# shanguanma/speaker_diarization

Hardware: AMD Instinct MI355X
Metric: diarized frames/sec (10 ms hop) (higher is better)
Workload: dtype bf16; 1 GPU; C2: AliMeeting-shaped 4-spk meeting, TS-VAD CAM++_ots_vad + 6-layer Conformer + BiLSTM (ots_vad_style v1), rs_len 6 s, shift 1 s; windows=600, global_batch=64, device_batch=640, parallelism=1 GPU

## Files before the change

### speaker_diarization_amd/csrc/mha_block.hip

```cpp
#include "common.h"
#include "kernels.h"
#include "launch.h"
#include "prof.h"

namespace sd {
namespace {

constexpr int kD = 384, kHD = 48, kNH = 8;
constexpr int kKT32 = kD / 32;
constexpr int kKC = kD / 64;
constexpr int kTP = 160;
constexpr int kTilesPerSeq = kTP / 16;
constexpr int kPR = 16;
constexpr int kSlot = kKC * kPR * 64;
constexpr int kDmaPerPiece = kKC * (kPR / 8);
constexpr int kVS = 48;
constexpr int kPieces = kNH * 3 * (kHD / kPR);
typedef __attribute__((address_space(3))) void* lds_ptr_t;

template <int SEQ, int W, int NSLOT, int QS>
struct MhaL {
  static constexpr int kTiles = SEQ * kTilesPerSeq;
  static constexpr int kMaxTiles = (kTiles + W - 1) / W;
  static constexpr int kThreads = W * 64;
  static constexpr int kSeqLds = 2 * kTP * QS + kTP * kVS;
  static constexpr size_t kSmem = sizeof(uint16_t) * ((size_t)NSLOT * kSlot + (size_t)SEQ * kSeqLds) +
                                  sizeof(float) * 3 * kD;
  static_assert(kMaxTiles == 2 || kMaxTiles == 3, "2 or 3 row tiles per wave (af registers)");
};

template <int N>
__device__ __forceinline__ void wait_vm() {
  asm volatile("s_waitcnt vmcnt(%0)" ::"n"(N) : "memory");
}

template <int SEQ, int W, int NSLOT, int QS, int PROBE = 0>
__global__ __launch_bounds__(W * 64) void mha_block_kernel(MhaBlockArgs a) {
  using L = MhaL<SEQ, W, NSLOT, QS>;
  constexpr int kTiles = L::kTiles, kMaxTiles = L::kMaxTiles, kThreads = L::kThreads, kSeqLds = L::kSeqLds;
  extern __shared__ __attribute__((aligned(1024))) uint16_t sm[];
  uint16_t* Ws = sm;
  const int tid = threadIdx.x, lane = tid & 63;
  const int w = __builtin_amdgcn_readfirstlane(tid >> 6);
  const int l15 = lane & 15, lk = lane >> 4;
  float* s_bias = reinterpret_cast<float*>(Ws + NSLOT * kSlot + SEQ * kSeqLds);
  const int T = a.T;
  const int ntile = w < kTiles - (kMaxTiles - 1) * W ? kMaxTiles : kMaxTiles - 1;
  int sqj[kMaxTiles], rowj[kMaxTiles];
#pragma unroll
  for (int j = 0; j < kMaxTiles; ++j) {
    const int t = w + W * j;
    sqj[j] = min(t, kTiles - 1) / kTilesPerSeq;
    rowj[j] = (min(t, kTiles - 1) % kTilesPerSeq) * 16 + l15;
  }
  auto qimg = [&](int sq) { return Ws + NSLOT * kSlot + sq * kSeqLds; };

  const int lrow = lane >> 3, lch = lane & 7;
  auto issue_piece = [&](int i) {
    const int h = i / 9, c = (i / 3) % 3, ft = i % 3;
    uint16_t* slot = Ws + (i % NSLOT) * kSlot;
    for (int j = w; j < kDmaPerPiece; j += W) {
      const int kc = j >> 1, rg = j & 1;
      const int r = rg * 8 + lrow;
      const uint32_t off =
          (uint32_t)((((int64_t)(c * kD + h * kHD + ft * kPR + r)) * kD + kc * 64 + ((lch ^ (r & 7)) * 8)) * 2);
      dma_lds16(reinterpret_cast<const char*>(a.W) + off, (lds_ptr_t)(slot + ((size_t)kc * kPR + rg * 8) * 64));
    }
  };
  const int my_dma = (kDmaPerPiece - w + W - 1) / W;
#pragma unroll
  for (int i = 0; i < NSLOT - 1; ++i) issue_piece(i);
  for (int i = tid; i < 3 * kD; i += kThreads) s_bias[i] = a.bias[i];
  if constexpr (QS > kHD) {
    for (int i = tid; i < SEQ * kTP * 2; i += kThreads) {
      const int q = i / (kTP * 2), r = (i >> 1) % kTP, c = kHD + (i & 1) * 8;
      uint16_t* qs = Ws + NSLOT * kSlot + q * kSeqLds;
      *reinterpret_cast<uint4*>(qs + r * QS + c) = make_uint4(0u, 0u, 0u, 0u);
      *reinterpret_cast<uint4*>(qs + kTP * QS + r * QS + c) = make_uint4(0u, 0u, 0u, 0u);
    }
  }

  bf16x8 af[kMaxTiles][kKT32];
#pragma unroll
  for (int rt = 0; rt < kMaxTiles; ++rt) {
    const int row = rowj[rt];
    const int s = blockIdx.x * SEQ + sqj[rt];
    const bool live = rt < ntile && s < a.S && row < T;
    const int64_t r = (int64_t)s * T + row;
    const uint16_t* yr = a.y_tiled ? reinterpret_cast<const uint16_t*>(a.y) + (r >> 4) * (16 * kD) + ((r & 15) + 16 * lk) * 8
                                   : reinterpret_cast<const uint16_t*>(a.y) + r * kD + 8 * lk;
    const int ks = a.y_tiled ? 512 : 32;
#pragma unroll
    for (int kk = 0; kk < kKT32; ++kk)
      af[rt][kk] = __builtin_bit_cast(bf16x8, live ? *reinterpret_cast<const uint4*>(yr + ks * kk)
                                                   : make_uint4(0u, 0u, 0u, 0u));
  }

  int klenj[SEQ];
#pragma unroll
  for (int q = 0; q < SEQ; ++q) {
    const int s = blockIdx.x * SEQ + q;
    klenj[q] = s < a.S ? (a.key_len ? min(a.key_len[s], T) : T) : 0;
  }
  const int tr_off = ((4 * lk + (l15 >> 2)) * kVS + 4 * (l15 & 3)) * 2;
  typedef short v4s __attribute__((ext_vector_type(4)));
  typedef __attribute__((address_space(3))) v4s* lds_v4s_t;
  bool drain = true;

  for (int i = 0; i < kPieces; ++i) {
    if constexpr (NSLOT == 4) {
      if (drain || i + 1 >= kPieces) wait_vm<0>();
      else if (i + 2 >= kPieces) {
        if (my_dma == 3) wait_vm<3>(); else if (my_dma == 2) wait_vm<2>(); else wait_vm<1>();
      } else {
        if (my_dma == 3) wait_vm<6>(); else if (my_dma == 2) wait_vm<4>(); else wait_vm<2>();
      }
    } else if constexpr (NSLOT == 3) {
      if (drain || i + 1 >= kPieces) wait_vm<0>();
      else if (my_dma == 3) wait_vm<3>();
      else if (my_dma == 2) wait_vm<2>();
      else wait_vm<1>();
    } else {
      static_assert(NSLOT == 2, "ring depth");
      wait_vm<0>();
    }
    drain = false;
    __syncthreads();
    if (i + NSLOT - 1 < kPieces) issue_piece(i + NSLOT - 1);
    const int h = i / 9, c = (i / 3) % 3, ft = i % 3;
    const uint16_t* slot = Ws + (i % NSLOT) * kSlot;
    floatx4 acc[kMaxTiles];
#pragma unroll
    for (int rt = 0; rt < kMaxTiles; ++rt) acc[rt] = floatx4{0.f, 0.f, 0.f, 0.f};
    auto wfrag = [&](int kk) {
      const int kc = kk >> 1, cc = (kk & 1) * 4 + lk;
      return *reinterpret_cast<const bf16x8*>(slot + (kc * kPR + l15) * 64 + ((cc ^ (l15 & 7)) * 8));
    };
    constexpr int kWPD = 3;
    bf16x8 wq[kWPD];
#pragma unroll
    for (int q = 0; q < kWPD; ++q) wq[q] = wfrag(q);
#pragma unroll
    for (int kk = 0; kk < kKT32; ++kk) {
      const bf16x8 wcur = wq[kk % kWPD];
      if (kk + kWPD < kKT32) wq[kk % kWPD] = wfrag(kk + kWPD);
      if constexpr (PROBE & 2) {
        asm volatile("" :: "v"(wcur));
        continue;
      }
      acc[0] = __builtin_amdgcn_mfma_f32_16x16x32_bf16(wcur, af[0][kk], acc[0], 0, 0, 0);
      acc[1] = __builtin_amdgcn_mfma_f32_16x16x32_bf16(wcur, af[1][kk], acc[1], 0, 0, 0);
      if constexpr (kMaxTiles > 2) {
        if (W == 4 || ntile > 2) acc[2] = __builtin_amdgcn_mfma_f32_16x16x32_bf16(wcur, af[2][kk], acc[2], 0, 0, 0);
      }
      asm volatile("" ::: "memory");
    }
    const int ld = c == 2 ? kVS : QS;
    const int coff = c * kTP * QS;
    const float scl = c == 0 ? a.scale : 1.f;
    const int n0 = ft * 16 + 4 * lk;
    const float4 bv = *reinterpret_cast<const float4*>(s_bias + c * kD + h * kHD + n0);
#pragma unroll
    for (int rt = 0; rt < kMaxTiles; ++rt)
      if (rt < ntile)
        *reinterpret_cast<uint2*>(qimg(sqj[rt]) + coff + rowj[rt] * ld + n0) =
            make_uint2(pack_bf16x2((acc[rt][0] + bv.x) * scl, (acc[rt][1] + bv.y) * scl),
                       pack_bf16x2((acc[rt][2] + bv.z) * scl, (acc[rt][3] + bv.w) * scl));
    if (c != 2 || ft != 2 || (PROBE & 1)) continue;
    __syncthreads();

#pragma unroll 1
    for (int rt = 0; rt < ntile; ++rt) {
      const int row = rowj[rt];
      const int s = blockIdx.x * SEQ + sqj[rt];
      if (s >= a.S) continue;
      const uint16_t* Qs = qimg(sqj[rt]);
      const uint16_t* Ks = Qs + kTP * QS;
      const uint16_t* Vs = Ks + kTP * QS;
      const int klen = klenj[sqj[rt]];
      bf16x8 qf[2];
#pragma unroll
      for (int kc = 0; kc < 2; ++kc) qf[kc] = *reinterpret_cast<const bf16x8*>(Qs + row * QS + kc * 32 + lk * 8);
      if constexpr (QS == kHD) {
        if (lk >= 2) qf[1] = __builtin_bit_cast(bf16x8, make_uint4(0u, 0u, 0u, 0u));
      }
      floatx4 o[3] = {{0.f, 0.f, 0.f, 0.f}, {0.f, 0.f, 0.f, 0.f}, {0.f, 0.f, 0.f, 0.f}};
      float m_run = -INFINITY, l_run = 0.f;
      for (int k0 = 0; k0 < klen; k0 += 32) {
        floatx4 sc[2];
#pragma unroll
        for (int st = 0; st < 2; ++st) {
          floatx4 sacc = {0.f, 0.f, 0.f, 0.f};
#pragma unroll
          for (int kc = 0; kc < 2; ++kc) {
            const bf16x8 kf = *reinterpret_cast<const bf16x8*>(Ks + (k0 + st * 16 + l15) * QS + kc * 32 + lk * 8);
            sacc = __builtin_amdgcn_mfma_f32_16x16x32_bf16(kf, qf[kc], sacc, 0, 0, 0);
          }
          sc[st] = sacc;
        }
        float tmax = -INFINITY;
#pragma unroll
        for (int st = 0; st < 2; ++st)
#pragma unroll
          for (int r = 0; r < 4; ++r) {
            const int key = k0 + st * 16 + lk * 4 + r;
            const float v = key < klen ? sc[st][r] : -INFINITY;
            sc[st][r] = v;
            tmax = fmaxf(tmax, v);
          }
        tmax = fmaxf(tmax, __shfl_xor(tmax, 16, 64));
        tmax = fmaxf(tmax, __shfl_xor(tmax, 32, 64));
        const float m_new = fmaxf(m_run, tmax);
        const float alpha = (m_new == -INFINITY) ? 1.f : __expf(m_run - m_new);
        float psum = 0.f;
#pragma unroll
        for (int st = 0; st < 2; ++st)
#pragma unroll
          for (int r = 0; r < 4; ++r) {
            const float pv = (m_new == -INFINITY) ? 0.f : __expf(sc[st][r] - m_new);
            sc[st][r] = pv;
            psum += pv;
          }
        psum += __shfl_xor(psum, 16, 64);
        psum += __shfl_xor(psum, 32, 64);
        l_run = l_run * alpha + psum;
        m_run = m_new;
        bf16x8 pb;
#pragma unroll
        for (int j = 0; j < 8; ++j) pb[j] = (__bf16)sc[j >> 2][j & 3];
        const uint32_t vbase = (uint32_t)reinterpret_cast<uintptr_t>((__attribute__((address_space(3))) void*)Vs) +
                               (uint32_t)(k0 * kVS * 2) + (uint32_t)tr_off;
#pragma unroll
        for (int dt = 0; dt < 3; ++dt) {
          const v4s lo = __builtin_amdgcn_ds_read_tr16_b64_v4i16((lds_v4s_t)(uintptr_t)(vbase + dt * 32));
          const v4s hi = __builtin_amdgcn_ds_read_tr16_b64_v4i16((lds_v4s_t)(uintptr_t)(vbase + 16 * kVS * 2 + dt * 32));
          const bf16x8 va = __builtin_bit_cast(bf16x8, __builtin_shufflevector(lo, hi, 0, 1, 2, 3, 4, 5, 6, 7));
#pragma unroll
          for (int r = 0; r < 4; ++r) o[dt][r] *= alpha;
          o[dt] = __builtin_amdgcn_mfma_f32_16x16x32_bf16(va, pb, o[dt], 0, 0, 0);
        }
      }
      if (row < T) {
        const float inv = l_run > 0.f ? 1.f / l_run : 0.f;
        const int64_t r = (int64_t)s * T + row;
        uint16_t* ob = reinterpret_cast<uint16_t*>(a.out);
#pragma unroll
        for (int dt = 0; dt < 3; ++dt) {
          const int f = h * kHD + dt * 16 + 4 * lk;
          const int64_t off = a.out_tiled ? (((r >> 4) * kKT32 + (f >> 5)) * 64 + (r & 15) + 16 * ((f & 31) >> 3)) * 8 + (f & 7)
                                          : r * a.ldo + f;
          *reinterpret_cast<uint2*>(ob + off) =
              make_uint2(pack_bf16x2(o[dt][0] * inv, o[dt][1] * inv), pack_bf16x2(o[dt][2] * inv, o[dt][3] * inv));
        }
        drain = true;
      }
    }
  }
}

template <int SEQ, int W, int NSLOT, int QS, int PROBE = 0>
void launch_mha(const MhaBlockArgs& a, hipStream_t st) {
  using L = MhaL<SEQ, W, NSLOT, QS>;
  allow_dynamic_lds<&mha_block_kernel<SEQ, W, NSLOT, QS, PROBE>>((int)L::kSmem);
  hipLaunchKernelGGL((mha_block_kernel<SEQ, W, NSLOT, QS, PROBE>), dim3((a.S + SEQ - 1) / SEQ), dim3(L::kThreads),
                     L::kSmem, st, a);
}

}

bool mha_block_supported(int D, int nh, int T, bool bf16) {
  static const bool off = getenv("SDIAR_NO_MHA_BLOCK") != nullptr;
  return !off && bf16 && D == kD && nh == kNH && T >= 1 && T <= kTP;
}

void mha_block(const MhaBlockArgs& a, hipStream_t st, int variant) {
  SD_CHECK(mha_block_supported(kD, a.nh, a.T, true) && a.D == kD, kErrInvalid, "mha_block: unsupported shape");
  SD_CHECK(a.ldo % 4 == 0, kErrInvalid, "mha_block: output row stride must be a multiple of 4");
  SD_CHECK(!(a.out_tiled || a.y_tiled) || ((int64_t)a.S * a.T % 16 == 0 && a.ldo == kD), kErrInvalid,
           "mha_block: the tiled layouts need S * T % 16 == 0 and ldo == D");
  if (a.S <= 0) return;
  SD_CHECK(a.y != nullptr, kErrInvalid, "mha_block: y (LayerNorm'd bf16 rows) is required");
  const double rows = (double)a.S * a.T;
  const double flops = 2.0 * rows * 3 * kD * kD + 4.0 * a.S * (double)a.T * a.T * kD;
  const double bytes = rows * kD * (2.0 + 2.0) + 2.0 * 3 * kD * kD;
  ProfScope prof("mha_block", flops, bytes, st);
  const int var = variant >= 0 ? variant : 0;
  switch (var) {
    case 1: launch_mha<2, 8, 3, 64>(a, st); break;
    case 2: launch_mha<1, 4, 2, 64>(a, st); break;
    case 3: launch_mha<1, 4, 2, 48>(a, st); break;
    case 4: launch_mha<1, 4, 3, 48>(a, st); break;
    case 5: launch_mha<1, 8, 3, 64>(a, st); break;
    case 6: launch_mha<1, 8, 2, 48>(a, st); break;
    case 7: launch_mha<2, 8, 4, 48>(a, st); break;
    case 8: launch_mha<2, 8, 3, 48, 1>(a, st); break;
    case 9: launch_mha<2, 8, 3, 48, 2>(a, st); break;
    case 10: launch_mha<2, 8, 3, 48, 3>(a, st); break;
    default: launch_mha<2, 8, 3, 48>(a, st); break;
  }
  SD_LAUNCH_CHECK();
}

}
```

Before: 2.486 million frames/s.

## Replace online softmax with two-pass exact-max attention and software-pipelined K reads

The attention inner loop now makes a first pass computing QK^T scores only to find the exact row max. A second pass then recomputes the scores, exponentiates against that fixed max and accumulates PV without any per-block rescaling of the output or running sum. K fragment loads are software-pipelined one block ahead, and sched_group_barrier hints interleave the exp VALU work with the next QK MFMAs. The row-sum reduction is deferred to the end, and output addressing is simplified to 32-bit offsets from a per-block base. In exchange the QK MFMAs are done twice.

```diff
diff --git a/speaker_diarization_amd/csrc/mha_block.hip b/speaker_diarization_amd/csrc/mha_block.hip
--- a/speaker_diarization_amd/csrc/mha_block.hip
+++ b/speaker_diarization_amd/csrc/mha_block.hip
@@ -2,6 +2,8 @@
 #include "kernels.h"
 #include "launch.h"
 #include "prof.h"
+
+#include <type_traits>
 
 namespace sd {
 namespace {
@@ -105,6 +107,9 @@
   const int tr_off = ((4 * lk + (l15 >> 2)) * kVS + 4 * (l15 & 3)) * 2;
   typedef short v4s __attribute__((ext_vector_type(4)));
   typedef __attribute__((address_space(3))) v4s* lds_v4s_t;
+  const int64_t r0 = (int64_t)blockIdx.x * SEQ * T;
+  const int r0lo = a.out_tiled ? (int)(r0 & 15) : 0;
+  uint16_t* const obase = reinterpret_cast<uint16_t*>(a.out) + (a.out_tiled ? (r0 >> 4) * (16 * kD) : r0 * a.ldo);
   bool drain = true;
 
   for (int i = 0; i < kPieces; ++i) {
@@ -185,71 +190,120 @@
         if (lk >= 2) qf[1] = __builtin_bit_cast(bf16x8, make_uint4(0u, 0u, 0u, 0u));
       }
       floatx4 o[3] = {{0.f, 0.f, 0.f, 0.f}, {0.f, 0.f, 0.f, 0.f}, {0.f, 0.f, 0.f, 0.f}};
-      float m_run = -INFINITY, l_run = 0.f;
-      for (int k0 = 0; k0 < klen; k0 += 32) {
-        floatx4 sc[2];
-#pragma unroll
-        for (int st = 0; st < 2; ++st) {
-          floatx4 sacc = {0.f, 0.f, 0.f, 0.f};
-#pragma unroll
-          for (int kc = 0; kc < 2; ++kc) {
-            const bf16x8 kf = *reinterpret_cast<const bf16x8*>(Ks + (k0 + st * 16 + l15) * QS + kc * 32 + lk * 8);
-            sacc = __builtin_amdgcn_mfma_f32_16x16x32_bf16(kf, qf[kc], sacc, 0, 0, 0);
+      const uint32_t kbase = (uint32_t)reinterpret_cast<uintptr_t>((lds_ptr_t)Ks) + (uint32_t)(l15 * QS + lk * 8) * 2;
+      const uint32_t vbase = (uint32_t)reinterpret_cast<uintptr_t>((lds_ptr_t)Vs) + (uint32_t)tr_off;
+      constexpr uint32_t kKStep = 32 * QS * 2, kVStep = 32 * kVS * 2;
+      typedef __attribute__((address_space(3))) const bf16x8* lds_bf16x8_t;
+      auto kread = [&](uint32_t ka, bf16x8 (&kf)[4]) {
+#pragma unroll
+        for (int j = 0; j < 4; ++j) kf[j] = *(lds_bf16x8_t)(uintptr_t)(ka + (uint32_t)((j >> 1) * 16 * QS + (j & 1) * 32) * 2);
+      };
+      auto smfma = [&](const bf16x8 (&kf)[4], floatx4 (&sc)[2]) {
+#pragma unroll
+        for (int st = 0; st < 2; ++st)
+          sc[st] = __builtin_amdgcn_mfma_f32_16x16x32_bf16(kf[2 * st], qf[0], floatx4{0.f, 0.f, 0.f, 0.f}, 0, 0, 0);
+#pragma unroll
+        for (int st = 0; st < 2; ++st)
+          sc[st] = __builtin_amdgcn_mfma_f32_16x16x32_bf16(kf[2 * st + 1], qf[1], sc[st], 0, 0, 0);
+      };
+      auto mask = [&](int k0, floatx4 (&sc)[2]) {
+#pragma unroll
+        for (int st = 0; st < 2; ++st)
+#pragma unroll
+          for (int r = 0; r < 4; ++r) sc[st][r] = k0 + st * 16 + lk * 4 + r < klen ? sc[st][r] : -INFINITY;
+      };
+      float l_run = 0.f;
+      if (klen > 0) {
+        float m_row = -INFINITY;
+        auto rowmax = [&](const floatx4 (&sc)[2]) {
+#pragma unroll
+          for (int st = 0; st < 2; ++st)
+#pragma unroll
+            for (int r = 0; r < 4; ++r) m_row = fmaxf(m_row, sc[st][r]);
+        };
+        bf16x8 kf[4];
+        uint32_t ka = kbase;
+        kread(ka, kf);
+        int k0 = 0;
+        for (; k0 + 32 < klen; k0 += 32) {
+          floatx4 sc[2];
+          smfma(kf, sc);
+          ka += kKStep;
+          asm volatile("" : "+v"(ka));
+          kread(ka, kf);
+          rowmax(sc);
+        }
+        {
+          floatx4 sc[2];
+          smfma(kf, sc);
+          mask(k0, sc);
+          rowmax(sc);
+        }
+        m_row = fmaxf(m_row, __shfl_xor(m_row, 16, 64));
+        m_row = fmaxf(m_row, __shfl_xor(m_row, 32, 64));
+        const bool no_max = __any(m_row == -INFINITY) != 0;
+        floatx4 scn[2];
+        ka = kbase;
+        uint32_t va = vbase;
+        kread(ka, kf);
+        smfma(kf, scn);
+        auto step = [&](int k0, auto last) {
+          constexpr bool kLast = decltype(last)::value;
+          floatx4 sc[2] = {scn[0], scn[1]};
+          if constexpr (!kLast) {
+            ka += kKStep;
+            asm volatile("" : "+v"(ka));
+            kread(ka, kf);
           }
-          sc[st] = sacc;
-        }
-        float tmax = -INFINITY;
-#pragma unroll
-        for (int st = 0; st < 2; ++st)
-#pragma unroll
-          for (int r = 0; r < 4; ++r) {
-            const int key = k0 + st * 16 + lk * 4 + r;
-            const float v = key < klen ? sc[st][r] : -INFINITY;
-            sc[st][r] = v;
-            tmax = fmaxf(tmax, v);
+          bf16x8 vf[3];
+#pragma unroll
+          for (int dt = 0; dt < 3; ++dt) {
+            const v4s lo = __builtin_amdgcn_ds_read_tr16_b64_v4i16((lds_v4s_t)(uintptr_t)(va + dt * 32));
+            const v4s hi = __builtin_amdgcn_ds_read_tr16_b64_v4i16((lds_v4s_t)(uintptr_t)(va + 16 * kVS * 2 + dt * 32));
+            vf[dt] = __builtin_bit_cast(bf16x8, __builtin_shufflevector(lo, hi, 0, 1, 2, 3, 4, 5, 6, 7));
           }
-        tmax = fmaxf(tmax, __shfl_xor(tmax, 16, 64));
-        tmax = fmaxf(tmax, __shfl_xor(tmax, 32, 64));
-        const float m_new = fmaxf(m_run, tmax);
-        const float alpha = (m_new == -INFINITY) ? 1.f : __expf(m_run - m_new);
-        float psum = 0.f;
-#pragma unroll
-        for (int st = 0; st < 2; ++st)
-#pragma unroll
-          for (int r = 0; r < 4; ++r) {
-            const float pv = (m_new == -INFINITY) ? 0.f : __expf(sc[st][r] - m_new);
-            sc[st][r] = pv;
-            psum += pv;
-          }
-        psum += __shfl_xor(psum, 16, 64);
-        psum += __shfl_xor(psum, 32, 64);
-        l_run = l_run * alpha + psum;
-        m_run = m_new;
-        bf16x8 pb;
-#pragma unroll
-        for (int j = 0; j < 8; ++j) pb[j] = (__bf16)sc[j >> 2][j & 3];
-        const uint32_t vbase = (uint32_t)reinterpret_cast<uintptr_t>((__attribute__((address_space(3))) void*)Vs) +
-                               (uint32_t)(k0 * kVS * 2) + (uint32_t)tr_off;
-#pragma unroll
-        for (int dt = 0; dt < 3; ++dt) {
-          const v4s lo = __builtin_amdgcn_ds_read_tr16_b64_v4i16((lds_v4s_t)(uintptr_t)(vbase + dt * 32));
-          const v4s hi = __builtin_amdgcn_ds_read_tr16_b64_v4i16((lds_v4s_t)(uintptr_t)(vbase + 16 * kVS * 2 + dt * 32));
-          const bf16x8 va = __builtin_bit_cast(bf16x8, __builtin_shufflevector(lo, hi, 0, 1, 2, 3, 4, 5, 6, 7));
-#pragma unroll
-          for (int r = 0; r < 4; ++r) o[dt][r] *= alpha;
-          o[dt] = __builtin_amdgcn_mfma_f32_16x16x32_bf16(va, pb, o[dt], 0, 0, 0);
-        }
-      }
+          va += kVStep;
+          asm volatile("" : "+v"(va));
+          __builtin_amdgcn_sched_barrier(0);
+          if constexpr (kLast) mask(k0, sc);
+          bf16x8 pb;
+          auto pexp = [&](auto guarded) {
+#pragma unroll
+            for (int j = 0; j < 8; ++j) {
+              float pv = __expf(sc[j >> 2][j & 3] - m_row);
+              if constexpr (decltype(guarded)::value) pv = (m_row == -INFINITY) ? 0.f : pv;
+              l_run += pv;
+              pb[j] = (__bf16)pv;
+            }
+            if constexpr (!kLast) {
+              smfma(kf, scn);
+#pragma unroll
+              for (int q = 0; q < 4; ++q) {
+                __builtin_amdgcn_sched_group_barrier(0x8, 1, 0);
+                __builtin_amdgcn_sched_group_barrier(0x2, 9, 0);
+              }
+            }
+          };
+          if (no_max) pexp(std::true_type{}); else pexp(std::false_type{});
+          __builtin_amdgcn_sched_barrier(0);
+#pragma unroll
+          for (int dt = 0; dt < 3; ++dt) o[dt] = __builtin_amdgcn_mfma_f32_16x16x32_bf16(vf[dt], pb, o[dt], 0, 0, 0);
+        };
+        for (k0 = 0; k0 + 32 < klen; k0 += 32) step(k0, std::false_type{});
+        step(k0, std::true_type{});
+      }
+      l_run += __shfl_xor(l_run, 16, 64);
+      l_run += __shfl_xor(l_run, 32, 64);
       if (row < T) {
         const float inv = l_run > 0.f ? 1.f / l_run : 0.f;
-        const int64_t r = (int64_t)s * T + row;
-        uint16_t* ob = reinterpret_cast<uint16_t*>(a.out);
+        const int rr = sqj[rt] * T + row, g = r0lo + rr;
+        const uint32_t ro = a.out_tiled ? (uint32_t)(g >> 4) * (16 * kD) + ((g & 15) + 16 * (lk >> 1)) * 8 + 4 * (lk & 1)
+                                        : (uint32_t)rr * (uint32_t)a.ldo + 4 * lk;
 #pragma unroll
         for (int dt = 0; dt < 3; ++dt) {
-          const int f = h * kHD + dt * 16 + 4 * lk;
-          const int64_t off = a.out_tiled ? (((r >> 4) * kKT32 + (f >> 5)) * 64 + (r & 15) + 16 * ((f & 31) >> 3)) * 8 + (f & 7)
-                                          : r * a.ldo + f;
-          *reinterpret_cast<uint2*>(ob + off) =
+          const int F = h * kHD + dt * 16;
+          const uint32_t off = ro + (a.out_tiled ? (F >> 5) * 512 + ((F >> 4) & 1) * 256 : F);
+          *reinterpret_cast<uint2*>(obase + off) =
               make_uint2(pack_bf16x2(o[dt][0] * inv, o[dt][1] * inv), pack_bf16x2(o[dt][2] * inv, o[dt][3] * inv));
         }
         drain = true;
@@ -275,7 +329,8 @@
 
 void mha_block(const MhaBlockArgs& a, hipStream_t st, int variant) {
   SD_CHECK(mha_block_supported(kD, a.nh, a.T, true) && a.D == kD, kErrInvalid, "mha_block: unsupported shape");
-  SD_CHECK(a.ldo % 4 == 0, kErrInvalid, "mha_block: output row stride must be a multiple of 4");
+  SD_CHECK(a.ldo % 4 == 0 && a.ldo <= (1 << 20), kErrInvalid,
+           "mha_block: output row stride must be a multiple of 4, at most 2^20");
   SD_CHECK(!(a.out_tiled || a.y_tiled) || ((int64_t)a.S * a.T % 16 == 0 && a.ldo == kD), kErrInvalid,
            "mha_block: the tiled layouts need S * T % 16 == 0 and ldo == D");
   if (a.S <= 0) return;
```

Result: no change. 2.510 million frames/s (median of 6 runs) (+1.0%).
